# dohlee/diffab-pytorch

Measured on AMD Instinct MI355X. Metric: CDR-residue denoise-steps/sec (K=128 patch), higher is better.
Workload: dtype f32 (bf16x6 / fp16x3 split-precision products on the 16-bit matrix cores, fp32 accumulate; fp32-accurate, DESIGN section 4)

## Files before the change

### diffab-pytorch_amd/csrc/ipa_persistent.hip

```cpp
#include "common.h"
#include "denoiser_internal.h"
#define AT_STAMP_REALTIME 1
#include "ipa_attn_tile.h"
#include "proj_frames_h3_tile.h"
#include "rowgemm_h3_tile.h"
#include "mlp_chain_tile.h"

namespace diffab {

namespace {
constexpr size_t cmax(size_t a, size_t b) { return a > b ? a : b; }
constexpr size_t kModuleLdsBytes = cmax(cmax(ipa_attn_lds_bytes(8), static_cast<size_t>(kChainLdsBytes)),
                                        cmax(static_cast<size_t>(pjh3::PJ_LDS_BYTES), static_cast<size_t>(h3tile::lds_bytes<128>())));
constexpr size_t kXImageOffset = cmax(static_cast<size_t>(pjh3::PJ_LDS_BYTES), static_cast<size_t>(h3tile::lds_bytes<128>())) / 4;
static_assert(kXImageOffset * 4 + h3tile::y_lds_bytes<128>() <= kModuleLdsBytes, "module LDS: no room for the x image of the dense phases");
static_assert(kModuleLdsBytes <= 160 * 1024, "module LDS: one work-group per CU within gfx950's 160 KiB");
static_assert(kXImageOffset % 4 == 0, "x image: 16-byte aligned rows");

struct ModuleArgs {
  float* xa;
  float* xb;
  float* proj;
  float* feat;
  const float* pair;
  const float* esc;
  const int* ctx_of_row;
  const int* last_layer_rows;
  const float* R;
  const float* t;
  const char* planes;
  size_t layer_stride, pj_off, out_off, wis_off, small_off;
  unsigned long long* stamps;
  const float* emb_X;
  MlpChainSet emb, heads;
  int B, NL;
  int stagger_ticks, stagger_classes;
};
}

__device__ __forceinline__ int module_plan_word(const int* __restrict__ plan, const int idx) {
  int w;
  asm volatile("s_load_dword %0, %1, 0x0\n\ts_waitcnt lgkmcnt(0)" : "=s"(w) : "s"(plan + idx) : "memory");
  return w;
}

template <int KRES>
__global__ __launch_bounds__(512) void ipa_module_persistent_kernel(const ModuleArgs a) {
  extern __shared__ __attribute__((aligned(16))) float lds[];
  constexpr int K = KRES, NTILE = K / TI, DT = K / 128;
  static_assert(KRES == 128 || KRES == 256, "patch-resident module: K = 128 or 256");
  const int M = a.B * K;
  if (a.stagger_ticks > 0 && a.stagger_classes > 1) {
    const unsigned long long t0 = __builtin_amdgcn_s_memrealtime();
    const unsigned long long wait = static_cast<unsigned long long>((blockIdx.x >> 3) % a.stagger_classes) * a.stagger_ticks;
    while (__builtin_amdgcn_s_memrealtime() - t0 < wait) __builtin_amdgcn_s_sleep(32);
  }
  unsigned long long* pstamps = a.stamps ? a.stamps + static_cast<size_t>(a.B) * a.NL * NTILE * 64 : nullptr;
  auto pstamp = [&](int b, int l, int k) {
    if (pstamps != nullptr && threadIdx.x == 0) pstamps[(static_cast<size_t>(b) * a.NL + l) * 4 + k] = __builtin_amdgcn_s_memrealtime();
  };
#pragma unroll 1
  for (int b = blockIdx.x; b < a.B; b += gridDim.x) {
    if (a.emb_X != nullptr) {
#pragma unroll 1
      for (int dt = 0; dt < DT; ++dt) {
        int tid = threadIdx.x;
        asm volatile("" : "+v"(tid));
        chaintile::mlp_chain_tile(reinterpret_cast<__bf16*>(lds), tid, b * DT + dt, a.emb_X, 128, a.emb.c[0].planes[0], a.emb.c[0].planes[1],
                                  nullptr, a.emb.c[0].bias[0], a.emb.c[0].bias[1], nullptr, a.emb.c[0].bias_idx0, a.emb.c[0].bias_div0, 2, 128,
                                  a.xa, 128, M);
        asm volatile("s_waitcnt vmcnt(0)" ::: "memory");
        __syncthreads();
      }
    }
#pragma unroll 1
    for (int l = 0; l < a.NL; ++l) {
      const char* lp = a.planes + static_cast<size_t>(l) * a.layer_stride;
      const float* small = reinterpret_cast<const float*>(lp + a.small_off);
      const float* xin = (l & 1) ? a.xb : a.xa;
      float* xout = (l & 1) ? a.xa : a.xb;
      pstamp(b, l, 0);
#pragma unroll 1
      for (int dt = 0; dt < DT; ++dt) {
        int tid = threadIdx.x;
        asm volatile("" : "+v"(tid));
        if (KRES == 128) {
          if (l == 0) {
            float* xl = lds + kXImageOffset;
            for (int i = tid; i < 128 * 32; i += 512) {
              const int row = i >> 5, c4 = 4 * (i & 31);
              *reinterpret_cast<float4*>(xl + row * h3tile::Y_LDS_LD + c4) =
                  *reinterpret_cast<const float4*>(xin + (static_cast<int64_t>(b) * 128 + row) * 128 + c4);
            }
            __syncthreads();
          }
          pjh3::proj_frames_h3_tile<true, false, true, true>(reinterpret_cast<_Float16*>(lds), tid, b, 0, 1, nullptr,
                                                             reinterpret_cast<const _Float16*>(lp + a.pj_off),
                                                             reinterpret_cast<const float*>(lp + a.wis_off), a.R, a.t, a.proj, M, 0, 0, 0,
                                                             lds + kXImageOffset);
        } else {
          pjh3::proj_frames_h3_tile<true, false>(reinterpret_cast<_Float16*>(lds), tid, b * DT + dt, 0, 1, xin,
                                                 reinterpret_cast<const _Float16*>(lp + a.pj_off), reinterpret_cast<const float*>(lp + a.wis_off),
                                                 a.R, a.t, a.proj, M);
        }
        if (dt + 1 < DT) {
          asm volatile("s_waitcnt vmcnt(0)" ::: "memory");
          __syncthreads();
        }
      }
      asm volatile("s_waitcnt vmcnt(0)" ::: "memory");
      __syncthreads();
      pstamp(b, l, 1);
      const int* rows = l + 1 == a.NL ? a.last_layer_rows : nullptr;
      const int n_items = rows != nullptr ? module_plan_word(rows, b * (2 + NTILE)) : NTILE;
#pragma unroll 1
      for (int item = 0; item < n_items; ++item) {
        const int i0 = rows != nullptr ? module_plan_word(rows, b * (2 + NTILE) + 2 + item) : item * TI;
        ipa_attn_tile<8, (KRES > 128), true>(lds, b, i0, static_cast<unsigned>((b * a.NL + l) * NTILE + item), a.proj, a.pair, a.R, a.t, small,
                                             small + 512, a.feat, K / 128, a.stamps, a.esc, nullptr, nullptr, a.ctx_of_row);
        asm volatile("s_waitcnt vmcnt(0)" ::: "memory");
        __syncthreads();
      }
      pstamp(b, l, 2);
#pragma unroll 1
      for (int dt = 0; dt < DT; ++dt) {
        int tid = threadIdx.x;
        asm volatile("" : "+v"(tid));
        if (KRES == 128)
          h3tile::rowgemm128_h3_tile<false, 128, false, true>(reinterpret_cast<_Float16*>(lds), tid, b, a.feat, AF,
                                                              reinterpret_cast<const _Float16*>(lp + a.out_off),
                                                              reinterpret_cast<const float*>(lp + a.wis_off) + ANP, small + 576, nullptr, 0,
                                                              l + 1 == a.NL ? xout : nullptr, 128, M, AF, 0, nullptr, lds + kXImageOffset);
        else
          h3tile::rowgemm128_h3_tile<false, 128>(reinterpret_cast<_Float16*>(lds), tid, b * DT + dt, a.feat, AF,
                                                 reinterpret_cast<const _Float16*>(lp + a.out_off),
                                                 reinterpret_cast<const float*>(lp + a.wis_off) + ANP, small + 576, nullptr, 0, xout, 128, M, AF);
        if (dt + 1 < DT) {
          asm volatile("s_waitcnt vmcnt(0)" ::: "memory");
          __syncthreads();
        }
      }
      asm volatile("s_waitcnt vmcnt(0)" ::: "memory");
      __syncthreads();
      pstamp(b, l, 3);
    }
    if (a.emb_X != nullptr) {
      const float* xfin = (a.NL & 1) ? a.xb : a.xa;
#pragma unroll 1
      for (int hdt = 0; hdt < 3 * DT; ++hdt) {
        const int hd = hdt / DT, dt = hdt % DT;
        const unsigned hslabs =
            a.last_layer_rows != nullptr ? static_cast<unsigned>(module_plan_word(a.last_layer_rows, b * (2 + NTILE) + 1)) : ~0u;
        const unsigned tslabs = (hslabs >> (4 * dt)) & 15u;
        if (tslabs == 0) continue;
        int tid = threadIdx.x;
        asm volatile("" : "+v"(tid));
#define HSEL(f) (hd == 0 ? a.heads.c[0].f : hd == 1 ? a.heads.c[1].f : a.heads.c[2].f)
        chaintile::mlp_chain_tile<true>(reinterpret_cast<__bf16*>(lds), tid, b * DT + dt, xfin, 128, HSEL(planes[0]), HSEL(planes[1]), HSEL(planes[2]),
                                  HSEL(bias[0]), HSEL(bias[1]), HSEL(bias[2]), HSEL(bias_idx0), HSEL(bias_div0), 3, HSEL(n_out),
                                  hd == 0 ? a.heads.Y[0] : hd == 1 ? a.heads.Y[1] : a.heads.Y[2],
                                  hd == 0 ? a.heads.ldy[0] : hd == 1 ? a.heads.ldy[1] : a.heads.ldy[2], M, tslabs);
#undef HSEL
        asm volatile("s_waitcnt vmcnt(0)" ::: "memory");
        __syncthreads();
      }
      if (pstamps != nullptr && threadIdx.x == 0) pstamps[static_cast<size_t>(a.B) * a.NL * 4 + b] = __builtin_amdgcn_s_memrealtime();
    }
  }
}

namespace {
int g_stagger_ticks = 1000, g_stagger_classes = 8;
unsigned long long* g_module_stamps = nullptr;
}
void set_module_stagger(int ticks, int classes) {
  g_stagger_ticks = ticks;
  g_stagger_classes = classes;
}
void set_module_stamps(void* p) { g_module_stamps = static_cast<unsigned long long*>(p); }

bool ipa_module_persistent_supported(const diffab_dims* d) {
  return fast_path_supported(d) && (d->K == 128 || d->K == 256) && d->NL >= 1;
}

int launch_ipa_module_persistent(const diffab_dims* d, float* xa, float* xb, const float* R, const float* t, float* ws, const void* planes,
                                 const float* pair_planes, hipStream_t st, const float* emb_X, const MlpChainSet* emb,
                                 const MlpChainSet* heads, const int* ctx_of_row, int n_ctx, const int* last_layer_rows) {
  DIFFAB_REQUIRE(ipa_module_persistent_supported(d) && xa && xb && R && t && ws && planes && pair_planes, DIFFAB_ERR_ARG,
                 "ipa_module_persistent: unsupported operands");
  DIFFAB_REQUIRE((reinterpret_cast<uintptr_t>(last_layer_rows) & 3) == 0, DIFFAB_ERR_ARG,
                 "ipa_module_persistent: the row plan must be 4-byte aligned");
  const size_t rows = static_cast<size_t>(d->B) * d->K;
  ModuleArgs a{};
  a.xa = xa;
  a.xb = xb;
  a.proj = ws;
  a.feat = ws + rows * ANP;
  a.pair = pair_planes + 64;
  a.esc = pair_row_scales(d, pair_planes, n_ctx);
  a.ctx_of_row = ctx_of_row;
  a.last_layer_rows = last_layer_rows;
  a.R = R;
  a.t = t;
  a.planes = static_cast<const char*>(planes);
  a.layer_stride = ipa_layer_planes_bytes();
  a.pj_off = ipa_layer_h3_pj_offset();
  a.out_off = ipa_layer_h3_out_offset();
  a.wis_off = ipa_layer_h3_wis_offset();
  a.small_off = ipa_layer_small_offset();
  a.stamps = g_module_stamps;
  if (emb_X != nullptr) {
    DIFFAB_REQUIRE(emb && heads && d->D == 128 && (reinterpret_cast<uintptr_t>(emb_X) & 15) == 0, DIFFAB_ERR_ARG,
                   "ipa_module_persistent: the fused MLP phases need both chain sets");
    a.emb_X = emb_X;
    a.emb = *emb;
    a.heads = *heads;
  }
  a.B = d->B;
  a.NL = d->NL;
  a.stagger_ticks = g_stagger_ticks;
  a.stagger_classes = g_stagger_classes;
  int dev = 0, ncu = 256;
  if (hipGetDevice(&dev) == hipSuccess) (void)hipDeviceGetAttribute(&ncu, hipDeviceAttributeMultiprocessorCount, dev);
  const int grid = d->B < ncu ? d->B : ncu;
#define MODULE_LAUNCH(K_)                                                                                                       \
  do {                                                                                                                            \
    DIFFAB_HIP_CHECK(hipFuncSetAttribute(reinterpret_cast<const void*>(ipa_module_persistent_kernel<K_>),                         \
                                         hipFuncAttributeMaxDynamicSharedMemorySize, static_cast<int>(kModuleLdsBytes)));        \
    timer_begin(st);                                                                                                              \
    hipLaunchKernelGGL((ipa_module_persistent_kernel<K_>), dim3(grid), dim3(512), kModuleLdsBytes, st, a);                        \
    timer_end(st);                                                                                                                \
  } while (0)
  if (d->K == 128) MODULE_LAUNCH(128);
  else MODULE_LAUNCH(256);
#undef MODULE_LAUNCH
  DIFFAB_LAUNCH_CHECK();
  return DIFFAB_OK;
}

}
```

Before: 14.98 million.

## Fuse three output-head MLP chains into one slab pass per 32-row pair

For K=128, the tail of the persistent module now runs all three output-head MLP chains together on one or two active 32-row slabs at a time, with waves split across heads and column halves. This replaces the per-head, per-tile loop that re-staged the input and synchronised once per head. The input is split to bf16x3 in LDS once and shared by all three heads, and weights are double-buffered in registers with prefetch. The cost is higher register pressure from the weight fragments and accumulators, and a new code path with its own layout and synchronisation. It also adds a timestamp write at block start for profiling.

New measurement: 15.18 million (median of 6 runs). 1.01x the previous value.

```diff
diff --git a/diffab-pytorch_amd/csrc/ipa_persistent.hip b/diffab-pytorch_amd/csrc/ipa_persistent.hip
--- a/diffab-pytorch_amd/csrc/ipa_persistent.hip
+++ b/diffab-pytorch_amd/csrc/ipa_persistent.hip
@@ -5,6 +5,7 @@
 #include "proj_frames_h3_tile.h"
 #include "rowgemm_h3_tile.h"
 #include "mlp_chain_tile.h"
+#include "mlp_chain_slab.h"
 
 namespace diffab {
 
@@ -61,6 +62,7 @@
   };
 #pragma unroll 1
   for (int b = blockIdx.x; b < a.B; b += gridDim.x) {
+    if (pstamps != nullptr && threadIdx.x == 0) pstamps[static_cast<size_t>(a.B) * a.NL * 4 + a.B + b] = __builtin_amdgcn_s_memrealtime();
     if (a.emb_X != nullptr) {
 #pragma unroll 1
       for (int dt = 0; dt < DT; ++dt) {
@@ -146,6 +148,21 @@
     }
     if (a.emb_X != nullptr) {
       const float* xfin = (a.NL & 1) ? a.xb : a.xa;
+      if (KRES == 128 && a.last_layer_rows != nullptr) {
+        unsigned rest = static_cast<unsigned>(module_plan_word(a.last_layer_rows, b * (2 + NTILE) + 1)) & 15u;
+#pragma unroll 1
+        while (rest != 0) {
+          const int s0 = __builtin_ctz(rest);
+          rest &= rest - 1;
+          const int ns = rest != 0 ? 2 : 1;
+          const int s1 = rest != 0 ? __builtin_ctz(rest) : s0;
+          rest &= rest - 1;
+          int tid = threadIdx.x;
+          asm volatile("" : "+v"(tid));
+          chainslab::mlp_chain_slabs<3>(reinterpret_cast<__bf16*>(lds), tid, ns, b * 128 + 32 * s0, b * 128 + 32 * s1, xfin, 128, a.heads, M);
+        }
+        asm volatile("s_waitcnt vmcnt(0)" ::: "memory");
+      } else {
 #pragma unroll 1
       for (int hdt = 0; hdt < 3 * DT; ++hdt) {
         const int hd = hdt / DT, dt = hdt % DT;
@@ -163,6 +180,7 @@
 #undef HSEL
         asm volatile("s_waitcnt vmcnt(0)" ::: "memory");
         __syncthreads();
+      }
       }
       if (pstamps != nullptr && threadIdx.x == 0) pstamps[static_cast<size_t>(a.B) * a.NL * 4 + b] = __builtin_amdgcn_s_memrealtime();
     }
diff --git a/diffab-pytorch_amd/csrc/mlp_chain_slab.h b/diffab-pytorch_amd/csrc/mlp_chain_slab.h
--- /dev/null
+++ b/diffab-pytorch_amd/csrc/mlp_chain_slab.h
@@ -0,0 +1,213 @@
+#pragma once
+#include <hip/hip_runtime.h>
+#include <cstdint>
+
+#include "mlp_chain_tile.h"
+
+namespace diffab {
+namespace chainslab {
+using b6tile::BK;
+using b6tile::b6_off;
+using b6tile::split3;
+typedef float f32x4 __attribute__((ext_vector_type(4)));
+typedef __bf16 bf16x4 __attribute__((ext_vector_type(4)));
+typedef __bf16 bf16x8 __attribute__((ext_vector_type(8)));
+typedef float f32x16 __attribute__((ext_vector_type(16)));
+typedef const bf16x8 __attribute__((address_space(1)))* global_bf16x8_p;
+typedef const float __attribute__((address_space(1)))* global_float_p;
+typedef const f32x4 __attribute__((address_space(1)))* global_f32x4_p;
+
+constexpr int kSlabImage = 4 * 3 * 32 * BK;
+template <int NCH>
+constexpr int slab_lds_bytes() { return 2 * NCH * kSlabImage * 2; }
+static_assert(slab_lds_bytes<3>() <= kChainLdsBytes, "slab form: within the LDS of the chain tile");
+
+template <typename T>
+__device__ __forceinline__ T* sel3(int L, T* p0, T* p1, T* p2) {
+  const uintptr_t m0 = -static_cast<uintptr_t>(L == 0), m1 = -static_cast<uintptr_t>(L == 1), m2 = -static_cast<uintptr_t>(L >= 2);
+  return reinterpret_cast<T*>((reinterpret_cast<uintptr_t>(p0) & m0) | (reinterpret_cast<uintptr_t>(p1) & m1) |
+                              (reinterpret_cast<uintptr_t>(p2) & m2));
+}
+
+template <int NCH>
+__device__ __forceinline__ void mlp_chain_slabs(__bf16* cl, const int tid, const int ns, const int row0a, const int row0b,
+                                                const float* __restrict__ X, int ldx, const MlpChainSet& cs, int M) {
+  static_assert(NCH == 1 || NCH == 3, "slab form: one chain or three");
+#define SLAB_CSEL(k_, f) ((NCH == 1 || (k_) == 0) ? cs.c[0].f : (k_) == 1 ? cs.c[NCH > 1 ? 1 : 0].f : cs.c[NCH - 1].f)
+#define SLAB_YSEL(k_, f) ((NCH == 1 || (k_) == 0) ? cs.f[0] : (k_) == 1 ? cs.f[NCH > 1 ? 1 : 0] : cs.f[NCH - 1])
+  const int lane = tid & 63, l31 = lane & 31, hk = lane >> 5;
+  const int wv_u = __builtin_amdgcn_readfirstlane(tid >> 6);
+  const int nl = cs.c[0].nlayers;
+  const bool has_unit = wv_u < 2 * NCH;
+  const int ch = has_unit ? wv_u % NCH : 0, cw = has_unit ? wv_u / NCH : 0;
+  const __bf16 *const pl0 = SLAB_CSEL(ch, planes[0]), *const pl1 = SLAB_CSEL(ch, planes[1]), *const pl2 = SLAB_CSEL(ch, planes[2]);
+  const float *const bs0 = SLAB_CSEL(ch, bias[0]), *const bs1 = SLAB_CSEL(ch, bias[1]), *const bs2 = SLAB_CSEL(ch, bias[2]);
+  const int64_t* const bias_idx0 = SLAB_CSEL(ch, bias_idx0);
+  const int bias_div0 = SLAB_CSEL(ch, bias_div0), n_out = SLAB_CSEL(ch, n_out), ldy = SLAB_YSEL(ch, ldy);
+  float* const Y = SLAB_YSEL(ch, Y);
+#undef SLAB_CSEL
+#undef SLAB_YSEL
+  const int ntt_last = n_out - 64 * cw >= 64 ? 2 : n_out - 64 * cw <= 0 ? 0 : (n_out - 64 * cw + 31) >> 5;
+  const int n_steps = !has_unit ? 0 : ntt_last > 0 ? 4 * nl : 4 * (nl - 1);
+  auto w_of = [&](int s) -> const __bf16* {
+    s = s < n_steps ? s : n_steps - 1;
+    const int L = s >> 2;
+    const __bf16* W = sel3(L, pl0, pl1, pl2);
+    return W + (s & 3) * (3 * 128 * BK) + (64 * cw) * BK;
+  };
+  const unsigned w_lane = static_cast<unsigned>((l31 * BK + 8 * hk) * 2);
+  bf16x8 wf[2][2][2][3];
+  auto load_w = [&](int slot, const __bf16* src) {
+#pragma unroll
+    for (int tt = 0; tt < 2; ++tt)
+#pragma unroll
+      for (int ks = 0; ks < 2; ++ks)
+#pragma unroll
+        for (int p = 0; p < 3; ++p)
+          wf[slot][tt][ks][p] =
+              *(global_bf16x8_p)(reinterpret_cast<uintptr_t>(src + (p * 128 + 32 * tt) * BK + 16 * ks) + w_lane);
+  };
+  if (n_steps > 0) {
+    load_w(0, w_of(0));
+    load_w(1, w_of(1));
+  }
+  {
+    f32x4 xr[2][2];
+#pragma unroll
+    for (int j = 0; j < 2; ++j) {
+      if (j >= ns) continue;
+#pragma unroll
+      for (int i = 0; i < 2; ++i) {
+        const int q = tid + 512 * i;
+        int row = (j ? row0b : row0a) + (q >> 5);
+        row = row < M ? row : M - 1;
+        xr[j][i] = *reinterpret_cast<const f32x4*>(X + static_cast<int64_t>(row) * ldx + 4 * (q & 31));
+      }
+    }
+#pragma unroll
+    for (int j = 0; j < 2; ++j) {
+      if (j >= ns) continue;
+#pragma unroll
+      for (int i = 0; i < 2; ++i) {
+        const int q = tid + 512 * i, lrow = q >> 5, c4 = q & 31;
+        bf16x4 h, m, l;
+#pragma unroll
+        for (int e = 0; e < 4; ++e) {
+          __bf16 hh, mm, ll;
+          split3(xr[j][i][e], hh, mm, ll);
+          h[e] = hh; m[e] = mm; l[e] = ll;
+        }
+        __bf16* dst = cl + j * kSlabImage + (c4 >> 3) * (3 * 32 * BK) + b6_off(lrow, (c4 & 7) >> 1) + 4 * (c4 & 1);
+        *reinterpret_cast<bf16x4*>(dst) = h;
+        *reinterpret_cast<bf16x4*>(dst + 32 * BK) = m;
+        *reinterpret_cast<bf16x4*>(dst + 2 * 32 * BK) = l;
+      }
+    }
+  }
+  __syncthreads();
+  const int fx = (l31 >> 2) & 3;
+  constexpr int TA[6] = {1, 2, 0, 1, 0, 0}, TB[6] = {1, 0, 2, 0, 1, 0};
+#pragma unroll 1
+  for (int L = 0; L < nl; ++L) {
+    const bool last = L == nl - 1;
+    const int ntt = last ? ntt_last : 2;
+    const bool active = has_unit && ntt > 0;
+    f32x16 acc[2][2];
+    if (active) {
+#pragma unroll
+      for (int j = 0; j < 2; ++j)
+#pragma unroll
+        for (int tt = 0; tt < 2; ++tt)
+#pragma unroll
+          for (int r = 0; r < 16; ++r) acc[j][tt][r] = 0.f;
+      const __bf16* al = cl + (L == 0 ? 0 : ch * kSlabImage) + l31 * BK;
+      const int slab_stride = L == 0 ? kSlabImage : NCH * kSlabImage;
+#pragma unroll
+      for (int c = 0; c < 4; ++c) {
+#pragma unroll
+        for (int ks = 0; ks < 2; ++ks) {
+          const int so = 8 * ((2 * ks + hk) ^ fx);
+#pragma unroll
+          for (int j = 0; j < 2; ++j) {
+            if (j >= ns) continue;
+            bf16x8 a[3];
+#pragma unroll
+            for (int p = 0; p < 3; ++p)
+              a[p] = *reinterpret_cast<const bf16x8*>(al + j * slab_stride + c * (3 * 32 * BK) + (p * 32) * BK + so);
+            if (ntt == 2) {
+#pragma unroll
+              for (int term = 0; term < 6; ++term)
+#pragma unroll
+                for (int tt = 0; tt < 2; ++tt)
+                  acc[j][tt] = __builtin_amdgcn_mfma_f32_32x32x16_bf16(wf[c & 1][tt][ks][TB[term]], a[TA[term]], acc[j][tt], 0, 0, 0);
+            } else {
+#pragma unroll
+              for (int term = 0; term < 6; ++term)
+                acc[j][0] = __builtin_amdgcn_mfma_f32_32x32x16_bf16(wf[c & 1][0][ks][TB[term]], a[TA[term]], acc[j][0], 0, 0, 0);
+            }
+          }
+        }
+        load_w(c & 1, w_of(4 * L + c + 2));
+        __builtin_amdgcn_sched_barrier(0);
+      }
+    }
+    __syncthreads();
+    if (active) {
+      const bool table = L == 0 && (bias_idx0 != nullptr || bias_div0 > 0);
+      const float* bl0 = sel3(L, bs0, bs1, bs2);
+#pragma unroll
+      for (int j = 0; j < 2; ++j) {
+        if (j >= ns) continue;
+        int row = (j ? row0b : row0a) + l31;
+        asm volatile("" : "+v"(row));
+        global_float_p bl = (global_float_p)reinterpret_cast<uintptr_t>(bl0);
+        if (table) {
+          const int rc = row < M ? row : M - 1;
+          const int64_t bi = bias_idx0 ? bias_idx0[rc] : rc / bias_div0;
+          bl += bi * 128;
+        }
+        __bf16* img_out = cl + (j * NCH + ch) * kSlabImage;
+#pragma unroll
+        for (int tt = 0; tt < 2; ++tt) {
+          if (tt >= ntt) continue;
+#pragma unroll
+          for (int g4 = 0; g4 < 4; ++g4) {
+            const int col = 64 * cw + 32 * tt + 8 * g4 + 4 * hk;
+            f32x4 bv = {0.f, 0.f, 0.f, 0.f};
+            if (bl && (table || !last || col + 3 < n_out)) bv = *(global_f32x4_p)(bl + col);
+            else if (bl && col < n_out) {
+#pragma unroll
+              for (int e = 0; e < 4; ++e)
+                if (col + e < n_out) bv[e] = bl[col + e];
+            }
+            float o[4];
+#pragma unroll
+            for (int e = 0; e < 4; ++e) o[e] = acc[j][tt][4 * g4 + e] + bv[e];
+            if (last) {
+              if (row < M) {
+#pragma unroll
+                for (int e = 0; e < 4; ++e)
+                  if (col + e < n_out) Y[static_cast<int64_t>(row) * ldy + col + e] = o[e];
+              }
+            } else {
+              bf16x4 h, m, l;
+#pragma unroll
+              for (int e = 0; e < 4; ++e) {
+                __bf16 hh, mm, ll;
+                split3(fmaxf(o[e], 0.f), hh, mm, ll);
+                h[e] = hh; m[e] = mm; l[e] = ll;
+              }
+              __bf16* dst = img_out + (col >> 5) * (3 * 32 * BK) + b6_off(l31, (col & 31) >> 3) + (col & 7);
+              *reinterpret_cast<bf16x4*>(dst) = h;
+              *reinterpret_cast<bf16x4*>(dst + 32 * BK) = m;
+              *reinterpret_cast<bf16x4*>(dst + 2 * 32 * BK) = l;
+            }
+          }
+        }
+      }
+    }
+    if (!last) __syncthreads();
+  }
+}
+}
+}
```
